# Lukeasargen/Show-Attend-and-Tell-Pytorch-Lightning

Hardware: AMD Instinct MI355X
Metric: captions/sec (train step) at B=128, 256px, seq_len=22 (higher is better)
Workload: dtype bf16; 1 GPU; C2: resnet50 encoder_size=7 encoder_dim=512 vocab=6400 T=22, 128 images/GPU x R=5 captions, trainable encoder, Adam, full lengths, decoder_tf=always; global_batch_images=128, parallelism=dp1, grad_bucket_dtype=fp32

## Files before the change

show-attend-and-tell-pytorch-lightning_amd/csrc/api.hip:

```cpp
#include <stdarg.h>

#include "../../include/sat_hip.h"
#include "decoder.h"
#include "gemm.h"
#include "gemm_bf16_common.h"
#include "temperature.h"
#include "caption_score.h"

namespace sat {
static thread_local char g_err[512] = {0};
int& dev_switch(int which) {
    static int v[SW_COUNT] = {0 , getenv("SAT_NO_WGRAD3X3") ? !atoi(getenv("SAT_NO_WGRAD3X3")) : 1,
                              getenv("SAT_REDUCE_Z16") ? atoi(getenv("SAT_REDUCE_Z16")) : 1, getenv("SAT_WIDE_TILES") ? atoi(getenv("SAT_WIDE_TILES")) : 0,
                              getenv("SAT_BN_ONEPASS") ? atoi(getenv("SAT_BN_ONEPASS")) : 1,
                              getenv("SAT_BN_VPT") ? atoi(getenv("SAT_BN_VPT")) : 2,
                              getenv("SAT_ACC_PREFETCH") ? atoi(getenv("SAT_ACC_PREFETCH")) : 0};
    return v[which];
}
int& trace_launches() { static int on = getenv("SAT_TRACE_LAUNCH") ? 1 : 0; return on; }
char* last_error_buf() { return g_err; }
int fail(int code, const char* fmt, ...) {
    va_list ap; va_start(ap, fmt); vsnprintf(g_err, sizeof g_err, fmt, ap); va_end(ap);
    return code;
}
}

using namespace sat;

extern "C" {

int sat_abi_version(void) { return SAT_HIP_ABI_VERSION; }
int sat_debug_trace_launches(int32_t on) { sat::trace_launches() = on ? 1 : 0; return SAT_OK; }
int sat_debug_option(const char* name, int32_t value) {
    if (!name) return fail(SAT_EINVAL, "debug_option: null name");
    if (!strcmp(name, "wgrad3x3")) { dev_switch(SW_WGRAD3X3) = value; return SAT_OK; }
    if (!strcmp(name, "reduce_z16")) { dev_switch(SW_REDUCE_Z16) = value; return SAT_OK; }
    if (!strcmp(name, "acc_prefetch")) { dev_switch(SW_ACC_PREFETCH) = value; return SAT_OK; }
    if (!strcmp(name, "bn_vpt")) { dev_switch(SW_BN_VPT) = value; return SAT_OK; }
    if (!strcmp(name, "bn_onepass")) { dev_switch(SW_BN_ONEPASS) = value; return SAT_OK; }
    if (!strcmp(name, "wide_tiles")) { dev_switch(SW_WIDE_TILES) = value; return SAT_OK; }
    if (!strcmp(name, "glds_tile")) { glds_force_tile() = value; return SAT_OK; }
    if (!strcmp(name, "glds_stages8")) { glds_stages8() = value; return SAT_OK; }
    if (!strcmp(name, "glds_tall_k")) { glds_tall_k() = value; return SAT_OK; }
    if (!strcmp(name, "glds_tall_conv")) { glds_tall_conv() = value; return SAT_OK; }
    if (!strcmp(name, "tile_override")) { gemm_tile_override() = value; return SAT_OK; }
    return fail(SAT_EINVAL, "debug_option: unknown option %s", name);
}
const char* sat_last_error(void) { return last_error_buf(); }

static int gemm_from_desc(const sat_gemm_desc* d, const sat_gemm_types* t, void* stream);
int sat_gemm_f32(const sat_gemm_desc* d, void* stream) { return gemm_from_desc(d, nullptr, stream); }
int sat_gemm_ex(const sat_gemm_desc* d, const sat_gemm_types* t, void* stream) {
    if (!t) return fail(SAT_EINVAL, "sat_gemm_ex: null type descriptor");
    return gemm_from_desc(d, t, stream);
}
static int gemm_from_desc(const sat_gemm_desc* d, const sat_gemm_types* t, void* stream) {
    if (!d) return fail(SAT_EINVAL, "sat_gemm_f32: null descriptor");
    if (d->amode != A_ROW && d->amode != A_KMAJOR) return fail(SAT_EINVAL, "sat_gemm_f32: amode %d (dense modes only)", d->amode);
    if (d->bmode != B_ROW && d->bmode != B_KMAJOR) return fail(SAT_EINVAL, "sat_gemm_f32: bmode %d (dense modes only)", d->bmode);
    GemmArgs g;
    g.A = d->A; g.lda = d->lda; g.a_rows = d->a_rows; g.B = d->B; g.ldb = d->ldb; g.C = d->C; g.ldc = d->ldc; g.c_rows = d->c_rows;
    g.M = d->M; g.N = d->N; g.K = d->K; g.amode = d->amode; g.bmode = d->bmode; g.accumulate = d->accumulate; g.epi = d->epi;
    g.bias = d->bias; g.e0 = d->e0; g.lde0 = d->lde0; g.c0 = d->c0; g.c1 = d->c1; g.slab = d->slab; g.slab_elems = d->slab_elems;
    if (t) { g.a_bf16 = t->a_bf16; g.b_bf16 = t->b_bf16; g.c_bf16 = t->c_bf16; g.bf16_mfma = t->bf16_mfma; }
    return launch_gemm(g, (hipStream_t)stream);
}

size_t sat_decoder_workspace_bytes(const sat_decoder_dims* d) {
    if (check_dims(d) != SAT_OK) return 0;
    return decoder_workspace_bytes(*d);
}

static int check_params(const sat_decoder_dims* d, const sat_decoder_params* w, const char* what) {
    if (!w) return fail(SAT_EINVAL, "%s: null parameter struct", what);
    if (!w->embedding || !w->init_f_w || !w->init_f_b || !w->init_i_w || !w->init_i_b || !w->w_ih || !w->w_hh || !w->b_ih || !w->b_hh ||
        !w->att_enc || !w->att_dec || !w->att_f || !w->beta_w || !w->beta_b || !w->out_hidden || !w->out_w)
        return fail(SAT_EINVAL, "%s: null tensor in parameter struct", what);
    if (d->deep_output && !w->out_context) return fail(SAT_EINVAL, "%s: deep output needs output.context.weight", what);
    for (int l = 1; l < d->layers; ++l)
        if (!w->up_w_ih[l - 1] || !w->up_w_hh[l - 1] || !w->up_b_ih[l - 1] || !w->up_b_hh[l - 1])
            return fail(SAT_EINVAL, "%s: null tensor for LSTM layer %d", what, l);
    return SAT_OK;
}
static int check_batch(const sat_decoder_batch* b) {
    if (!b || !b->ann || !b->caps || !b->lengths || !b->prow || !b->src_row || !b->step_offsets_host || !b->teacher_host)
        return fail(SAT_EINVAL, "decoder: null field in batch struct");
    return SAT_OK;
}

int sat_decoder_train_fwd(const sat_decoder_dims* d, const sat_decoder_params* w, const sat_decoder_batch* b, float* logits_packed,
                          float* alphas, void* workspace, size_t workspace_bytes, void* stream) {
    SAT_TRY(check_dims(d)); SAT_TRY(check_params(d, w, "decoder_train_fwd")); SAT_TRY(check_batch(b));
    if (!alphas || !workspace || (d->P > 0 && !logits_packed)) return fail(SAT_EINVAL, "decoder_train_fwd: null output/workspace");
    return decoder_fwd(*d, *w, *b, logits_packed, alphas, (char*)workspace, workspace_bytes, (hipStream_t)stream);
}

int sat_decoder_train_bwd(const sat_decoder_dims* d, const sat_decoder_params* w, const sat_decoder_batch* b, const float* dlogits_packed,
                          const float* alphas, const float* dalphas, const sat_decoder_params* g, float* dann, void* workspace,
                          size_t workspace_bytes, void* stream) {
    SAT_TRY(check_dims(d)); SAT_TRY(check_params(d, w, "decoder_train_bwd")); SAT_TRY(check_params(d, g, "decoder_train_bwd(grads)")); SAT_TRY(check_batch(b));
    if (!alphas || !dann || !workspace || (d->P > 0 && !dlogits_packed)) return fail(SAT_EINVAL, "decoder_train_bwd: null input/output/workspace");
    return decoder_bwd(*d, *w, *b, dlogits_packed, alphas, dalphas, *g, dann, (char*)workspace, workspace_bytes, (hipStream_t)stream);
}

int sat_decoder_train_bwd_fork(const sat_decoder_dims* d, const sat_decoder_params* w, const sat_decoder_batch* b, const float* dlogits_packed,
                               const float* alphas, const float* dalphas, const sat_decoder_params* g, float* dann, void* workspace,
                               size_t workspace_bytes, void* side_stream, void* event, void* stream) {
    SAT_TRY(check_dims(d)); SAT_TRY(check_params(d, w, "decoder_train_bwd_fork")); SAT_TRY(check_params(d, g, "decoder_train_bwd_fork(grads)")); SAT_TRY(check_batch(b));
    if (!alphas || !dann || !workspace || (d->P > 0 && !dlogits_packed)) return fail(SAT_EINVAL, "decoder_train_bwd_fork: null input/output/workspace");
    if ((side_stream != nullptr) != (event != nullptr)) return fail(SAT_EINVAL, "decoder_train_bwd_fork: side stream and event go together (got %s only)", side_stream ? "a stream" : "an event");
    if (side_stream && side_stream == stream) return fail(SAT_EINVAL, "decoder_train_bwd_fork: the side stream is the caller's stream");
    if (workspace_bytes < decoder_workspace_bytes(*d))
        return fail(SAT_EINVAL, "decoder_train_bwd_fork: workspace %zu < %zu bytes", workspace_bytes, decoder_workspace_bytes(*d));
    return decoder_bwd(*d, *w, *b, dlogits_packed, alphas, dalphas, *g, dann, (char*)workspace, workspace_bytes, (hipStream_t)stream, (hipStream_t)side_stream,
                       (hipEvent_t)event);
}

int sat_decoder_train_bwd_reg(const sat_decoder_dims* d, const sat_decoder_params* w, const sat_decoder_batch* b, const float* dlogits_packed,
                              const float* alphas, const float* dalphas, const sat_decoder_params* g, float* dann, void* workspace,
                              size_t workspace_bytes, void* side_stream, void* event, void* stream, const float* reg_gscale) {
    if (!reg_gscale)
        return sat_decoder_train_bwd_fork(d, w, b, dlogits_packed, alphas, dalphas, g, dann, workspace, workspace_bytes, side_stream, event, stream);
    SAT_TRY(check_dims(d)); SAT_TRY(check_params(d, w, "decoder_train_bwd_reg")); SAT_TRY(check_params(d, g, "decoder_train_bwd_reg(grads)")); SAT_TRY(check_batch(b));
    if (!alphas || !dann || !workspace || (d->P > 0 && !dlogits_packed)) return fail(SAT_EINVAL, "decoder_train_bwd_reg: null input/output/workspace");
    if ((side_stream != nullptr) != (event != nullptr)) return fail(SAT_EINVAL, "decoder_train_bwd_reg: side stream and event go together (got %s only)", side_stream ? "a stream" : "an event");
    if (side_stream && side_stream == stream) return fail(SAT_EINVAL, "decoder_train_bwd_reg: the side stream is the caller's stream");
    if (workspace_bytes < decoder_workspace_bytes(*d))
        return fail(SAT_EINVAL, "decoder_train_bwd_reg: workspace %zu < %zu bytes", workspace_bytes, decoder_workspace_bytes(*d));
    return decoder_bwd(*d, *w, *b, dlogits_packed, alphas, dalphas, *g, dann, (char*)workspace, workspace_bytes, (hipStream_t)stream, (hipStream_t)side_stream,
                       (hipEvent_t)event, reg_gscale);
}

int sat_decoder_train_reg_fwd(const sat_decoder_dims* d, const sat_decoder_batch* b, void* workspace, size_t workspace_bytes, void* scratch, float* out,
                              void* stream) {
    SAT_TRY(check_dims(d)); SAT_TRY(check_batch(b));
    if (!workspace || !scratch || !out) return fail(SAT_EINVAL, "decoder_train_reg_fwd: null workspace/scratch/out");
    if (workspace_bytes < decoder_workspace_bytes(*d))
        return fail(SAT_EINVAL, "decoder_train_reg_fwd: workspace %zu < %zu bytes", workspace_bytes, decoder_workspace_bytes(*d));
    return decoder_reg_fwd(*d, *b, (char*)workspace, workspace_bytes, scratch, out, (hipStream_t)stream);
}

static int check_activation_reg(const char* what, const void* hidden, const void* lengths, const void* p2, const char* n2, const void* p3, const char* n3,
                                int32_t N, int32_t T1, int32_t n, int64_t P, int64_t Q) {
    if (!hidden || !lengths || !p2 || !p3)
        return fail(SAT_EINVAL, "%s: null pointer (%s)", what, !hidden ? "hidden" : !lengths ? "lengths" : !p2 ? n2 : n3);
    if (N <= 0 || T1 <= 0 || n <= 0) return fail(SAT_EINVAL, "%s: non-positive size (N=%d T1=%d n=%d)", what, N, T1, n);
    if (P < 0 || Q < 0 || Q > P || P > (int64_t)N * T1)
        return fail(SAT_EINVAL, "%s: live counts P=%lld Q=%lld outside 0 <= Q <= P <= N*T1=%lld", what, (long long)P, (long long)Q, (long long)N * T1);
    return SAT_OK;
}
size_t sat_activation_reg_scratch_bytes(int32_t N, int32_t T1, int32_t n) {
    if (N <= 0 || T1 <= 0 || n <= 0) { fail(SAT_EINVAL, "activation_reg_scratch_bytes: non-positive size (N=%d T1=%d n=%d)", N, T1, n); return 0; }
    return activation_reg_scratch_bytes(N, T1, n);
}
int sat_activation_reg_fwd(const float* hidden, const int32_t* lengths, int32_t N, int32_t T1, int32_t n, int64_t P, int64_t Q, void* scratch, float* out,
                           void* stream) {
    SAT_TRY(check_activation_reg("activation_reg_fwd", hidden, lengths, scratch, "scratch", out, "out", N, T1, n, P, Q));
    return activation_reg_fwd(hidden, lengths, N, T1, n, (long)P, (long)Q, scratch, out, (hipStream_t)stream);
}
int sat_activation_reg_bwd(const float* hidden, const int32_t* lengths, int32_t N, int32_t T1, int32_t n, int64_t P, int64_t Q, const float* gscale, float* dH,
                           void* stream) {
    SAT_TRY(check_activation_reg("activation_reg_bwd", hidden, lengths, gscale, "gscale", dH, "dH", N, T1, n, P, Q));
    return activation_reg_bwd(hidden, lengths, N, T1, n, (long)P, (long)Q, gscale, dH, (hipStream_t)stream);
}

int sat_ce_label_smooth_fwd(const float* logits, const int32_t* targets, int32_t P, int32_t V, float smoothing, float* lse_rows,
                            float* loss_rows, int32_t* correct_rows, float* out, void* stream) {
    if (!logits || !targets || !lse_rows || !loss_rows || !correct_rows || !out) return fail(SAT_EINVAL, "ce_label_smooth_fwd: null pointer");
    return ce_fwd(logits, targets, P, V, smoothing, lse_rows, loss_rows, correct_rows, out, (hipStream_t)stream);
}
int sat_ce_label_smooth_bwd(const float* logits, const int32_t* targets, const float* lse_rows, int32_t P, int32_t V, float smoothing,
                            const float* gscale, float* dlogits, void* stream) {
    if (!logits || !targets || !lse_rows || !dlogits) return fail(SAT_EINVAL, "ce_label_smooth_bwd: null pointer");
    return ce_bwd(logits, targets, lse_rows, P, V, smoothing, gscale, dlogits, (hipStream_t)stream);
}
int sat_doubly_stochastic_fwd(const float* alphas, int32_t N, int32_t T1, int32_t L, float gamma, float* asum, float* part, float* out, void* stream) {
    if (!alphas || !asum || !part || !out) return fail(SAT_EINVAL, "doubly_stochastic_fwd: null pointer");
    return ds_fwd(alphas, N, T1, L, gamma, asum, part, out, (hipStream_t)stream);
}
int sat_doubly_stochastic_bwd(const float* asum, const float* gscale, int32_t N, int32_t T1, int32_t L, float gamma, float* dalphas, void* stream) {
    if (!asum || !dalphas) return fail(SAT_EINVAL, "doubly_stochastic_bwd: null pointer");
    return ds_bwd(asum, gscale, N, T1, L, gamma, dalphas, (hipStream_t)stream);
}

size_t sat_temperature_workspace_bytes(int32_t P, int32_t V) {
    if (P <= 0 || V <= 0) { fail(SAT_EINVAL, "temperature_workspace_bytes: non-positive size (P=%d V=%d)", P, V); return 0; }
    return temperature_workspace_bytes(P, V);
// ... 480 lines not shown
```

show-attend-and-tell-pytorch-lightning_amd/csrc/gemm.h:

```cpp
#pragma once
#include "common.h"

namespace sat {

enum AMode : int {
    A_ROW = 0,
    A_KMAJOR = 1,
    A_CONV_FWD = 2,
    A_CONV_DGRAD = 3
};
enum BMode : int {
    B_ROW = 0,
    B_KMAJOR = 1,
    B_CONV_WGRAD = 2,
    B_CONV_DGRAD_W = 3
};
enum Epi : int {
    EPI_NONE = 0,
    EPI_BIAS = 1,
    EPI_BIAS_SIGMOID_RANGE = 2,
    EPI_ADD_TANH = 3,
    EPI_MUL_DTANH = 4,
    EPI_BIAS_RELU = 5
};

struct ConvGeom {
    int N, H, W, C;
    int K, R, S;
    int P, Q;
    int stride, pad;
    int sw = 0;
    int cls = 0, ph = 0, pw = 0, Hc = 0, Wc = 0, r0 = 0, rc = 0, s0 = 0, sc = 0;
};

struct GemmArgs {
    const void* A = nullptr; long lda = 0; const int* a_rows = nullptr;
    const void* B = nullptr; long ldb = 0;
    void* C = nullptr;        long ldc = 0; const int* c_rows = nullptr;
    int a_bf16 = 0, b_bf16 = 0, c_bf16 = 0;
    int bf16_mfma = 0;
    int M = 0, N = 0, K = 0;
    int amode = A_ROW, bmode = B_ROW;
    int accumulate = 0;
    int epi = EPI_NONE;
    const float* bias = nullptr;
    const float* e0 = nullptr; long lde0 = 0;
    int c0 = 0, c1 = 0;
    ConvGeom g = {};
    float* slab = nullptr; long slab_elems = 0;
    const void* bn_x = nullptr; const unsigned char* bn_mask = nullptr; const float* bn_mean = nullptr; const float* bn_invstd = nullptr;
    const void* add_src = nullptr; const unsigned char* add_mask = nullptr;
    float* tile_stats = nullptr; int* tile_rows = nullptr;
};

int launch_gemm(const GemmArgs& a, hipStream_t stream);
int launch_gemm_bf16(const GemmArgs& a, hipStream_t stream);
int gemm_bf16_eligible(const GemmArgs& a);
enum { SW_UNUSED0 = 0, SW_WGRAD3X3 = 1, SW_REDUCE_Z16 = 2, SW_WIDE_TILES = 3, SW_BN_ONEPASS = 4, SW_BN_VPT = 5, SW_ACC_PREFETCH = 6, SW_COUNT = 7 };
int& dev_switch(int which);

int wgrad3x3_eligible(const ConvGeom& g);
int launch_wgrad3x3(const void* dy, const void* x, float* dw, const ConvGeom& g, float* slab, long slab_elems, hipStream_t st);
size_t gemm_slab_bytes(int M, int N, int K);

}
```

show-attend-and-tell-pytorch-lightning_amd/csrc/gemm_bf16_common.h:

```cpp
#pragma once
#include <stdlib.h>

#include "gemm.h"

namespace sat {

typedef __bf16 bf16x8 __attribute__((ext_vector_type(8)));
typedef __bf16 bf16x4 __attribute__((ext_vector_type(4)));
typedef short s16x4 __attribute__((ext_vector_type(4)));
typedef float f32x16 __attribute__((ext_vector_type(16)));

constexpr int NT = 256;

struct BArgs {
    const void* A; long lda; const int* a_rows;
    const void* B; long ldb;
    void* C; long ldc; const int* c_rows;
    int M, N, K;
    int accumulate, epi;
    const float* bias; const float* e0; long lde0; int c0, c1;
    ConvGeom g;
    int kchunk, nsplit;
    float* slab;
    int wide_store;
// ... 321 lines not shown
        __syncthreads();
        constexpr int VPR = BN / 8;
#pragma unroll
        for (int j = 0; j < BM * VPR / NTH; ++j) {
            int v = tid + j * NTH, lr = v / VPR, lc = (v % VPR) * 8;
            int row = bm + lr, col = bn + lc;
            if (row < a.M && col < a.N) {
                bf16x8 o = *reinterpret_cast<const bf16x8*>(cs + lr * LDC + lc);
                const long orow = a.g.cls ? class_row(a, row) : (long)row;
                __bf16* dst = reinterpret_cast<__bf16*>(a.C) + orow * a.ldc + col;
                if (a.accumulate) {
                    const long off = orow * a.ldc + col;
                    bf16x8 old = *reinterpret_cast<const bf16x8*>((a.add_src ? a.add_src : reinterpret_cast<const __bf16*>(a.C)) + off);
                    const unsigned mb = a.add_mask ? (unsigned)a.add_mask[off >> 3] : 0xFFu;
#pragma unroll
                    for (int e = 0; e < 8; ++e) o[e] = (__bf16)((float)o[e] + (((mb >> e) & 1u) ? (float)old[e] : 0.f));
                }
                *reinterpret_cast<bf16x8*>(dst) = o;
                bacc.add(j, o);
            }
        }
        bacc.finish(a, reinterpret_cast<float*>(smem + BM * LDC), bm / BM, bn, tid);
        return;
    }
    if ((a.nsplit > 1) ? a.wide_slab : (sizeof(TC) == 4 && a.wide_store)) {
        constexpr int LDF = BN + 4, RB = BM / WR, VPR = BN / 4;
        float* fs = reinterpret_cast<float*>(smem);
#pragma unroll
        for (int h = 0; h < WR; ++h) {
            __syncthreads();
            if (wrow == h) {
#pragma unroll
                for (int i = 0; i < TM; ++i)
#pragma unroll
                    for (int j = 0; j < TN; ++j)
#pragma unroll
                        for (int r = 0; r < 16; ++r)
                            fs[(i * 32 + (r & 3) + 8 * (r >> 2) + 4 * lh) * LDF + wn + j * 32 + li] = acc[i][j][r];
            }
            __syncthreads();
#pragma unroll
            for (int jj = 0; jj < RB * VPR / NTH; ++jj) {
                const int v = tid + jj * NTH, lr = v / VPR, lc = (v % VPR) * 4;
                const int row = bm + h * RB + lr, col = bn + lc;
                if (row < a.M && col < a.N) {
                    float4 o = *reinterpret_cast<const float4*>(fs + lr * LDF + lc);
                    if (a.nsplit > 1) { *reinterpret_cast<float4*>(a.slab + ((long)bz * a.M + row) * a.N + col) = o; continue; }
                    const long orow = a.g.cls ? class_row(a, row) : (long)row;
                    float* dst = reinterpret_cast<float*>(a.C) + orow * a.ldc + col;
                    if (a.accumulate) { const float4 old = *reinterpret_cast<const float4*>(dst); o.x += old.x; o.y += old.y; o.z += old.z; o.w += old.w; }
                    if (a.epi != EPI_NONE) {
                        o.x = ep_value(a, row, col, o.x); o.y = ep_value(a, row, col + 1, o.y);
                        o.z = ep_value(a, row, col + 2, o.z); o.w = ep_value(a, row, col + 3, o.w);
                    }
                    *reinterpret_cast<float4*>(dst) = o;
                }
            }
        }
        return;
    }
#pragma unroll
    for (int i = 0; i < TM; ++i)
#pragma unroll
        for (int j = 0; j < TN; ++j)
#pragma unroll
            for (int r = 0; r < 16; ++r) {
                int row = bm + wm + i * 32 + (r & 3) + 8 * (r >> 2) + 4 * lh;
                int col = bn + wn + j * 32 + li;
                if (row < a.M && col < a.N) {
                    if (a.nsplit > 1) a.slab[((long)bz * a.M + row) * a.N + col] = acc[i][j][r];
                    else put<TC>(a, row, col, acc[i][j][r]);
                }
            }
}

template <typename TC>
__global__ void splitk_reduce_b_kernel(BArgs a) {
    long idx = (long)blockIdx.x * blockDim.x + threadIdx.x;
    long total = (long)a.M * a.N;
    if (idx >= total) return;
    float v = 0.f;
    for (int z = 0; z < a.nsplit; ++z) v += a.slab[(long)z * total + idx];
    put<TC>(a, (int)(idx / a.N), (int)(idx % a.N), v);
}
template <typename TC>
__global__ void splitk_reduce_b4_kernel(BArgs a) {
    const long idx4 = (long)blockIdx.x * blockDim.x + threadIdx.x;
    const long total4 = (long)a.M * a.N / 4;
    if (idx4 >= total4) return;
    float4 v = make_float4(0.f, 0.f, 0.f, 0.f);
    const float4* s4 = reinterpret_cast<const float4*>(a.slab);
#pragma unroll 4
    for (int z = 0; z < a.nsplit; ++z) { const float4 t = s4[(long)z * total4 + idx4]; v.x += t.x; v.y += t.y; v.z += t.z; v.w += t.w; }
    const long e = idx4 * 4; const int row = (int)(e / a.N), col = (int)(e % a.N);
    if (sizeof(TC) == 4 && a.wide_store && !a.g.cls) {
        float* dst = reinterpret_cast<float*>(a.C) + (long)row * a.ldc + col;
        if (a.accumulate) { const float4 old = *reinterpret_cast<const float4*>(dst); v.x += old.x; v.y += old.y; v.z += old.z; v.w += old.w; }
        if (a.epi != EPI_NONE) { v.x = ep_value(a, row, col, v.x); v.y = ep_value(a, row, col + 1, v.y); v.z = ep_value(a, row, col + 2, v.z); v.w = ep_value(a, row, col + 3, v.w); }
        *reinterpret_cast<float4*>(dst) = v;
    } else {
        put<TC>(a, row, col, v.x); put<TC>(a, row, col + 1, v.y); put<TC>(a, row, col + 2, v.z); put<TC>(a, row, col + 3, v.w);
    }
}

template <typename TC>
__global__ __launch_bounds__(256) void splitk_reduce_z16_kernel(BArgs a) {
    __shared__ float4 part[16][16];
    const int ev = threadIdx.x & 15, zl = threadIdx.x >> 4;
    const long idx4 = (long)blockIdx.x * 16 + ev;
    const long total4 = (long)a.M * a.N / 4;
    float4 v = make_float4(0.f, 0.f, 0.f, 0.f);
    if (idx4 < total4) {
        const float4* s4 = reinterpret_cast<const float4*>(a.slab);
#pragma unroll 4
        for (int z = zl; z < a.nsplit; z += 16) { const float4 t = s4[(long)z * total4 + idx4]; v.x += t.x; v.y += t.y; v.z += t.z; v.w += t.w; }
    }
    part[zl][ev] = v;
    __syncthreads();
    if (zl != 0 || idx4 >= total4) return;
#pragma unroll
    for (int l = 1; l < 16; ++l) { const float4 t = part[l][ev]; v.x += t.x; v.y += t.y; v.z += t.z; v.w += t.w; }
    const long e = idx4 * 4; const int row = (int)(e / a.N), col = (int)(e % a.N);
    if (sizeof(TC) == 4 && a.wide_store && !a.g.cls) {
        float* dst = reinterpret_cast<float*>(a.C) + (long)row * a.ldc + col;
        if (a.accumulate) { const float4 old = *reinterpret_cast<const float4*>(dst); v.x += old.x; v.y += old.y; v.z += old.z; v.w += old.w; }
        if (a.epi != EPI_NONE) { v.x = ep_value(a, row, col, v.x); v.y = ep_value(a, row, col + 1, v.y); v.z = ep_value(a, row, col + 2, v.z); v.w = ep_value(a, row, col + 3, v.w); }
        *reinterpret_cast<float4*>(dst) = v;
    } else {
        put<TC>(a, row, col, v.x); put<TC>(a, row, col + 1, v.y); put<TC>(a, row, col + 2, v.z); put<TC>(a, row, col + 3, v.w);
    }
}

template <typename TC>
inline int launch_splitk_reduce(const BArgs& k, hipStream_t st) {
    const long total = (long)k.M * k.N;
    const int z16 = dev_switch(SW_REDUCE_Z16);
    if (k.wide_slab && z16 && k.nsplit >= 32 && total / 4 / 256 < 256)
        hipLaunchKernelGGL(splitk_reduce_z16_kernel<TC>, dim3(cdiv(total / 4, 16)), dim3(256), 0, st, k);
    else if (k.wide_slab) hipLaunchKernelGGL(splitk_reduce_b4_kernel<TC>, dim3(cdiv(total / 4, 256)), dim3(256), 0, st, k);
    else hipLaunchKernelGGL(splitk_reduce_b_kernel<TC>, dim3(cdiv(total, 256)), dim3(256), 0, st, k);
    return launch_ok("splitk_reduce_b");
}

__device__ __forceinline__ void xcd_tile(int& bx, int& by, int& bz, int y_fastest = 0) {
    const unsigned total = gridDim.x * gridDim.y * gridDim.z;
    const unsigned orig = (blockIdx.z * gridDim.y + blockIdx.y) * gridDim.x + blockIdx.x;
    const unsigned q = total >> 3, r = total & 7, xcd = orig & 7, idx = orig >> 3;
    const unsigned lin = (xcd < r ? xcd * (q + 1) : r * (q + 1) + (xcd - r) * q) + idx;
    if (y_fastest) { by = lin % gridDim.y; const unsigned t2 = lin / gridDim.y; bx = t2 % gridDim.x; bz = t2 / gridDim.x; }
    else { bx = lin % gridDim.x; const unsigned t2 = lin / gridDim.x; by = t2 % gridDim.y; bz = t2 / gridDim.y; }
}

int launch_gemm_glds(const BArgs& k, int amode, int bmode, int c_bf16, int BMt, hipStream_t st, int* bm_used = nullptr);
int& glds_force_tile();
int& glds_stages8();
int& glds_tall_k();
int& glds_tall_conv();
int& glds_ablate();
int& gemm_tile_override();

}
```

show-attend-and-tell-pytorch-lightning_amd/csrc/gemm_glds.hip:

```cpp
#include <stdlib.h>

#include "gemm_bf16_common.h"

namespace sat {

template <int AM, int BMo, typename TC> int glds_run_64(const BArgs& k, hipStream_t st);
template <int AM, int BMo, typename TC> int glds_run_128(const BArgs& k, hipStream_t st);
template <int AM, int BMo, typename TC> int glds_run_128x64(const BArgs& k, hipStream_t st);
#ifdef SAT_DEV_TILES
template <int AM, int BMo, typename TC> int glds_run_256x128(const BArgs& k, hipStream_t st);
template <int AM, int BMo, typename TC> int glds_run_256(const BArgs& k, hipStream_t st);
#endif

enum { TILE_64 = 0, TILE_128 = 1, TILE_128x64 = 2, TILE_256x128 = 3, TILE_256 = 4 };
template <int AM, int BMo, typename TC>
static int rung_tiles(const BArgs& k, int tile, hipStream_t st, int* bm_used) {
    switch (tile) {
#ifdef SAT_DEV_TILES
        case TILE_256: if (bm_used) *bm_used = 256; return glds_run_256<AM, BMo, TC>(k, st);
        case TILE_256x128: if (bm_used) *bm_used = 256; return glds_run_256x128<AM, BMo, TC>(k, st);
#else
        case TILE_256: case TILE_256x128: return -1;
#endif
        case TILE_128: if (bm_used) *bm_used = 128; return glds_run_128<AM, BMo, TC>(k, st);
        case TILE_128x64: if (bm_used) *bm_used = 128; return glds_run_128x64<AM, BMo, TC>(k, st);
        default: if (bm_used) *bm_used = 64; return glds_run_64<AM, BMo, TC>(k, st);
    }
}

int& glds_force_tile() { static int v = getenv("SAT_GLDS_TILE") ? atoi(getenv("SAT_GLDS_TILE")) : -1; return v; }
int& glds_ablate() { static int v = 0; return v; }
int& glds_tall_k() { static int v = getenv("SAT_GLDS_TALL_K") ? atoi(getenv("SAT_GLDS_TALL_K")) : 1 << 30; return v; }
int& glds_tall_conv() { static int v = getenv("SAT_GLDS_TALL_CONV") ? atoi(getenv("SAT_GLDS_TALL_CONV")) : 1152; return v; }
int& glds_stages8() { static int v = getenv("SAT_GLDS_STAGES8") ? atoi(getenv("SAT_GLDS_STAGES8")) : 0; return v; }

int launch_gemm_glds(const BArgs& k0, int amode, int bmode, int c_bf16, int BMt, hipStream_t st, int* bm_used) {
    const int force_tile = glds_force_tile();
    static const int off = getenv("SAT_NO_GLDS") ? atoi(getenv("SAT_NO_GLDS")) : 0;
    static const int force_stages = getenv("SAT_GLDS_STAGES") ? atoi(getenv("SAT_GLDS_STAGES")) : 0;
    static const int deep_from = getenv("SAT_GLDS_DEEP_FROM") ? atoi(getenv("SAT_GLDS_DEEP_FROM")) : 1 << 30;
    static const int rotate = getenv("SAT_GLDS_ROT") ? atoi(getenv("SAT_GLDS_ROT")) : 1 << 20;
    if (off) return -1;
    BArgs k = k0;
    const int ktiles = cdiv(k.kchunk < k.K ? k.kchunk : k.K, 64);
    static const int s1_upto = getenv("SAT_GLDS_S1_UPTO") ? atoi(getenv("SAT_GLDS_S1_UPTO")) : 1 << 30;
    k.nstage = force_stages ? force_stages : (ktiles >= deep_from ? 4 : ((ktiles == 1 || (c_bf16 && ktiles <= s1_upto)) ? 1 : 2));
    k.rotate = rotate;
    if (k.nstage < 1) k.nstage = 1;
    if (k.nstage > 4) k.nstage = 4;
    static const int tall = getenv("SAT_GLDS_TALL") ? atoi(getenv("SAT_GLDS_TALL")) : 2;
    int tile = (BMt >= 256) ? (BMt == 256 ? TILE_256 : TILE_256x128) : (BMt == 128 ? TILE_128 : TILE_64);
    if (tile == TILE_64 && tall && bmode != B_CONV_WGRAD && k.N <= 64 && (amode == A_KMAJOR ? (tall > 1 && k.M >= 128) : k.M >= 8192)) tile = TILE_128x64;
    static const int tall_conv_tiles = getenv("SAT_GLDS_TALL_CONV_TILES") ? atoi(getenv("SAT_GLDS_TALL_CONV_TILES")) : 512;
    if (tile == TILE_128 && bmode != B_CONV_WGRAD && k.nsplit <= 1 &&
        ((amode == A_ROW && k.K <= glds_tall_k()) || ((amode == A_CONV_FWD || amode == A_CONV_DGRAD) && (k.K <= glds_tall_conv() || (long)cdiv(k.M, 128) * cdiv(k.N, 128) < tall_conv_tiles)))) tile = TILE_128x64;
    if (force_tile >= 0) tile = force_tile;
    if (tile == TILE_256 || tile == TILE_256x128) {
        const int maxs = (tile == TILE_256) ? 2 : 3;
        const int deep8 = glds_stages8();
        if (ktiles > 1) k.nstage = deep8 ? (deep8 < maxs ? deep8 : maxs) : (ktiles >= 3 ? maxs : 2);
    }
    {
        static const int order = getenv("SAT_TILE_ORDER") ? atoi(getenv("SAT_TILE_ORDER")) : -1;
        const int tbm = (tile == TILE_64) ? 64 : 128, tbn = (tile == TILE_128) ? 128 : 64;
        const int mt = cdiv(k.M, tbm), nt = cdiv(k.N, tbn);
        k.y_fastest = order >= 0 ? order : (amode == A_ROW && bmode != B_CONV_WGRAD && mt <= 16 && nt >= 2 * mt);
    }
    const ConvGeom& g = k.g;
    if (g.sw && g.sw != g.stride) return -1;
    if (k.K % 64 || k.kchunk % 64 || k.a_rows) return -1;
    if (amode == A_CONV_FWD && (g.C % 64 || g.R * g.S > 32)) return -1;
    if (amode == A_CONV_DGRAD && (g.K % 64 || g.R * g.S > 32 || (g.stride != 1 && !g.cls))) return -1;
    if (bmode == B_CONV_WGRAD && g.R * g.S > 32) return -1;
    const long lim = 1L << 30;
    long a_el = 0, b_el = 0;
    switch (amode) {
        case A_ROW: a_el = (long)k.M * k.lda; break;
        case A_KMAJOR: a_el = (long)k.K * k.lda; break;
        case A_CONV_FWD: a_el = (long)g.N * g.H * g.W * g.C; break;
        default: a_el = (long)g.N * g.P * g.Q * g.K; break;
    }
    switch (bmode) {
        case B_ROW: b_el = (long)k.N * k.ldb; break;
        case B_KMAJOR: b_el = (long)k.K * k.ldb; break;
        case B_CONV_WGRAD: b_el = (long)g.N * g.H * g.W * g.C; break;
        default: b_el = (long)g.K * g.R * g.S * g.C; break;
    }
    if (a_el >= lim || b_el >= lim) return -1;
    if ((amode == A_KMAJOR && k.M < 8) || (bmode != B_ROW && k.N < 8)) return -1;
#define SAT_GCASE(AMV, BMV, TC) return rung_tiles<AMV, BMV, TC>(k, tile, st, bm_used);
    if (amode == A_CONV_FWD && bmode == B_ROW && c_bf16) SAT_GCASE(A_CONV_FWD, B_ROW, __bf16)
    if (amode == A_ROW && bmode == B_ROW && c_bf16) SAT_GCASE(A_ROW, B_ROW, __bf16)
    if (amode == A_ROW && bmode == B_ROW && !c_bf16) SAT_GCASE(A_ROW, B_ROW, float)
    if (amode == A_CONV_DGRAD && bmode == B_CONV_DGRAD_W && c_bf16) SAT_GCASE(A_CONV_DGRAD, B_CONV_DGRAD_W, __bf16)
    if (amode == A_ROW && bmode == B_KMAJOR && c_bf16) SAT_GCASE(A_ROW, B_KMAJOR, __bf16)
    if (amode == A_ROW && bmode == B_KMAJOR && !c_bf16) SAT_GCASE(A_ROW, B_KMAJOR, float)
    if (amode == A_KMAJOR && bmode == B_CONV_WGRAD && !c_bf16) SAT_GCASE(A_KMAJOR, B_CONV_WGRAD, float)
    if (amode == A_KMAJOR && bmode == B_KMAJOR && !c_bf16) SAT_GCASE(A_KMAJOR, B_KMAJOR, float)
#undef SAT_GCASE
    return -1;
}

}
```

Before: 32680 captions/s.

## Add intra-block wave split-K GEMM kernel for small fp32 output GEMMs

Result: no change. 32990 captions/s (median of 6 runs) (+1.0%).

```diff
diff --git a/show-attend-and-tell-pytorch-lightning_amd/csrc/api.hip b/show-attend-and-tell-pytorch-lightning_amd/csrc/api.hip
--- a/show-attend-and-tell-pytorch-lightning_amd/csrc/api.hip
+++ b/show-attend-and-tell-pytorch-lightning_amd/csrc/api.hip
@@ -10,7 +10,7 @@
 namespace sat {
 static thread_local char g_err[512] = {0};
 int& dev_switch(int which) {
-    static int v[SW_COUNT] = {0 , getenv("SAT_NO_WGRAD3X3") ? !atoi(getenv("SAT_NO_WGRAD3X3")) : 1,
+    static int v[SW_COUNT] = {getenv("SAT_GLDS_WAVE_SPLIT") ? atoi(getenv("SAT_GLDS_WAVE_SPLIT")) : 1, getenv("SAT_NO_WGRAD3X3") ? !atoi(getenv("SAT_NO_WGRAD3X3")) : 1,
                               getenv("SAT_REDUCE_Z16") ? atoi(getenv("SAT_REDUCE_Z16")) : 1, getenv("SAT_WIDE_TILES") ? atoi(getenv("SAT_WIDE_TILES")) : 0,
                               getenv("SAT_BN_ONEPASS") ? atoi(getenv("SAT_BN_ONEPASS")) : 1,
                               getenv("SAT_BN_VPT") ? atoi(getenv("SAT_BN_VPT")) : 2,
@@ -33,6 +33,7 @@
 int sat_debug_trace_launches(int32_t on) { sat::trace_launches() = on ? 1 : 0; return SAT_OK; }
 int sat_debug_option(const char* name, int32_t value) {
     if (!name) return fail(SAT_EINVAL, "debug_option: null name");
+    if (!strcmp(name, "wave_split")) { dev_switch(SW_WAVE_SPLIT) = value; return SAT_OK; }
     if (!strcmp(name, "wgrad3x3")) { dev_switch(SW_WGRAD3X3) = value; return SAT_OK; }
     if (!strcmp(name, "reduce_z16")) { dev_switch(SW_REDUCE_Z16) = value; return SAT_OK; }
     if (!strcmp(name, "acc_prefetch")) { dev_switch(SW_ACC_PREFETCH) = value; return SAT_OK; }
diff --git a/show-attend-and-tell-pytorch-lightning_amd/csrc/gemm.h b/show-attend-and-tell-pytorch-lightning_amd/csrc/gemm.h
--- a/show-attend-and-tell-pytorch-lightning_amd/csrc/gemm.h
+++ b/show-attend-and-tell-pytorch-lightning_amd/csrc/gemm.h
@@ -56,7 +56,7 @@
 int launch_gemm(const GemmArgs& a, hipStream_t stream);
 int launch_gemm_bf16(const GemmArgs& a, hipStream_t stream);
 int gemm_bf16_eligible(const GemmArgs& a);
-enum { SW_UNUSED0 = 0, SW_WGRAD3X3 = 1, SW_REDUCE_Z16 = 2, SW_WIDE_TILES = 3, SW_BN_ONEPASS = 4, SW_BN_VPT = 5, SW_ACC_PREFETCH = 6, SW_COUNT = 7 };
+enum { SW_WAVE_SPLIT = 0, SW_WGRAD3X3 = 1, SW_REDUCE_Z16 = 2, SW_WIDE_TILES = 3, SW_BN_ONEPASS = 4, SW_BN_VPT = 5, SW_ACC_PREFETCH = 6, SW_COUNT = 7 };
 int& dev_switch(int which);
 
 int wgrad3x3_eligible(const ConvGeom& g);
diff --git a/show-attend-and-tell-pytorch-lightning_amd/csrc/gemm_bf16_common.h b/show-attend-and-tell-pytorch-lightning_amd/csrc/gemm_bf16_common.h
--- a/show-attend-and-tell-pytorch-lightning_amd/csrc/gemm_bf16_common.h
+++ b/show-attend-and-tell-pytorch-lightning_amd/csrc/gemm_bf16_common.h
@@ -497,6 +497,8 @@
 }
 
 int launch_gemm_glds(const BArgs& k, int amode, int bmode, int c_bf16, int BMt, hipStream_t st, int* bm_used = nullptr);
+constexpr int WAVE_SPLIT_ROWS = 32;
+int glds_run_wave_split(const BArgs& k, hipStream_t st);
 int& glds_force_tile();
 int& glds_stages8();
 int& glds_tall_k();
diff --git a/show-attend-and-tell-pytorch-lightning_amd/csrc/gemm_glds.hip b/show-attend-and-tell-pytorch-lightning_amd/csrc/gemm_glds.hip
--- a/show-attend-and-tell-pytorch-lightning_amd/csrc/gemm_glds.hip
+++ b/show-attend-and-tell-pytorch-lightning_amd/csrc/gemm_glds.hip
@@ -33,6 +33,14 @@
 int& glds_tall_k() { static int v = getenv("SAT_GLDS_TALL_K") ? atoi(getenv("SAT_GLDS_TALL_K")) : 1 << 30; return v; }
 int& glds_tall_conv() { static int v = getenv("SAT_GLDS_TALL_CONV") ? atoi(getenv("SAT_GLDS_TALL_CONV")) : 1152; return v; }
 int& glds_stages8() { static int v = getenv("SAT_GLDS_STAGES8") ? atoi(getenv("SAT_GLDS_STAGES8")) : 0; return v; }
+static int cu_count() {
+    static const int n = [] {
+        int dev = 0, v = 0;
+        if (hipGetDevice(&dev) != hipSuccess || hipDeviceGetAttribute(&v, hipDeviceAttributeMultiprocessorCount, dev) != hipSuccess) v = 0;
+        return v;
+    }();
+    return n;
+}
 
 int launch_gemm_glds(const BArgs& k0, int amode, int bmode, int c_bf16, int BMt, hipStream_t st, int* bm_used) {
     const int force_tile = glds_force_tile();
@@ -88,6 +96,11 @@
     }
     if (a_el >= lim || b_el >= lim) return -1;
     if ((amode == A_KMAJOR && k.M < 8) || (bmode != B_ROW && k.N < 8)) return -1;
+    if (dev_switch(SW_WAVE_SPLIT) && tile == TILE_64 && amode == A_ROW && bmode == B_KMAJOR && !c_bf16 && !k.c_rows && !g.cls && !k.tile_stats &&
+        k.nsplit >= 2 && k.nsplit <= 4 && k.wide_slab && k.wide_store && (long)cdiv(k.M, WAVE_SPLIT_ROWS) * cdiv(k.N, 64) <= cu_count()) {
+        if (bm_used) *bm_used = 64;
+        return glds_run_wave_split(k, st);
+    }
 #define SAT_GCASE(AMV, BMV, TC) return rung_tiles<AMV, BMV, TC>(k, tile, st, bm_used);
     if (amode == A_CONV_FWD && bmode == B_ROW && c_bf16) SAT_GCASE(A_CONV_FWD, B_ROW, __bf16)
     if (amode == A_ROW && bmode == B_ROW && c_bf16) SAT_GCASE(A_ROW, B_ROW, __bf16)
diff --git a/show-attend-and-tell-pytorch-lightning_amd/csrc/gemm_glds_t64ws.hip b/show-attend-and-tell-pytorch-lightning_amd/csrc/gemm_glds_t64ws.hip
--- /dev/null
+++ b/show-attend-and-tell-pytorch-lightning_amd/csrc/gemm_glds_t64ws.hip
@@ -0,0 +1,222 @@
+#include "gemm_glds_kernel.h"
+
+namespace sat {
+
+__device__ __forceinline__ unsigned lds_addr(const void* p) { return (unsigned)(size_t)(lptr_t)p; }
+__device__ __forceinline__ bf16x8 lds_read_b128(const __bf16* p) {
+    bf16x8 v = {};
+#if defined(__HIP_DEVICE_COMPILE__)
+    asm volatile("ds_read_b128 %0, %1" : "=v"(v) : "v"(lds_addr(p)));
+#endif
+    return v;
+}
+__device__ __forceinline__ bf16x4 lds_read_tr16_b64(const __bf16* p) {
+    bf16x4 v = {};
+#if defined(__HIP_DEVICE_COMPILE__)
+    asm volatile("ds_read_b64_tr_b16 %0, %1" : "=v"(v) : "v"(lds_addr(p)));
+#endif
+    return v;
+}
+__device__ __forceinline__ void lds_reads_done() { asm volatile("s_waitcnt lgkmcnt(0)" ::: "memory"); }
+template <typename T> __device__ __forceinline__ void lds_use(T& v) {
+#if defined(__HIP_DEVICE_COMPILE__)
+    asm volatile("" : "+v"(v));
+#endif
+}
+
+template <int BM, int S>
+__global__ __launch_bounds__(256, 1) void gemm_glds_ws_kernel(BArgs a) {
+    constexpr int KB = 64, BN = 64;
+    constexpr int A_EL = BM * KB, B_EL = BN * KB, STAGE = A_EL + B_EL;
+    constexpr int NA = BM / 8, NB = BN / 8, G = NA + NB;
+    constexpr int TM = BM / 32, TN = 2;
+    constexpr int LDF = BN + 4;
+    static_assert(BM * LDF * 4 <= S * STAGE * 2, "the fp32 tile is staged in the wave's own ring");
+    static_assert(S == 2 || S == 3, "ring depth");
+    extern __shared__ __attribute__((aligned(1024))) __bf16 smem[];
+
+    const int tid = threadIdx.x, lane = tid & 63;
+    const int z = __builtin_amdgcn_readfirstlane(tid >> 6);
+    int bx, by, bz;
+    xcd_tile(bx, by, bz, a.y_fastest);
+    const int bm = by * BM, bn = bx * BN;
+    const int kbeg = z * a.kchunk;
+    const int kend = min(a.K, kbeg + a.kchunk);
+    const int li = lane & 31, lh = lane >> 5;
+    const int tg = lane >> 4, ti = lane & 15;
+    const int t_h = tg >> 1, t_mh = tg & 1, t_q = ti >> 2, t_p = ti & 3;
+    const i32x4 rA = make_rsrc(a.A), rB = make_rsrc(a.B);
+    __bf16* ring = smem + z * S * STAGE;
+    const int by64 = (by * BM) >> 6;
+
+    int a_off0[NA], b_off0[NB];
+#pragma unroll
+    for (int j = 0; j < NA; ++j) {
+        const int row = j * 8 + (lane >> 3), ks = (lane & 7) ^ ((row >> 1) & 7);
+        int m = bm + row;
+        if (m >= a.M) m = a.M - 1;
+        a_off0[j] = (int)(((long)m * a.lda + ks * 8) * 2);
+    }
+#pragma unroll
+    for (int j = 0; j < NB; ++j) {
+        const int krow = j * 8 + (lane >> 3), sl = lane & 7;
+        const int lq = (sl >> 2) ^ ((krow >> 1) & 1);
+        int n = bn + (lq * 4 + (sl & 3)) * 8;
+        if (n >= a.N) n = a.N - 8;
+        b_off0[j] = (int)(((long)krow * a.ldb + n) * 2);
+    }
+
+    const int T = (kend - kbeg + KB - 1) / KB;
+    int tcur = (T > 0 && a.rotate) ? (int)((unsigned)(bx * 5 + by64 * 3 + z) % (unsigned)(T < a.rotate ? T : a.rotate)) : 0;
+    int sA = 0, sB = 0;
+    auto seek = [&](int tile) {
+        const int k0 = kbeg + tile * KB;
+        sA = k0 * 2;
+        sB = (int)((long)k0 * a.ldb * 2);
+    };
+    seek(tcur);
+    auto advance_tile = [&]() {
+        if (++tcur == T) { tcur = 0; seek(0); return; }
+        sA += KB * 2;
+        sB += (int)(KB * a.ldb * 2);
+    };
+    auto issue_piece = [&](int buf, int jj) {
+        __bf16* as = ring + buf * STAGE; __bf16* bs = as + A_EL;
+#pragma unroll
+        for (int j = 0; j < NA; ++j) if (j == jj) dma16(rA, a_off0[j], sA, as + j * 512);
+#pragma unroll
+        for (int j = 0; j < NB; ++j) if (j + NA == jj) dma16(rB, b_off0[j], sB, bs + j * 512);
+    };
+
+    f32x16 acc[TM][TN];
+#pragma unroll
+    for (int i = 0; i < TM; ++i)
+#pragma unroll
+        for (int j = 0; j < TN; ++j)
+#pragma unroll
+            for (int r = 0; r < 16; ++r) acc[i][j][r] = 0.f;
+
+    int a_off[TM], a_sw[TM], b_off[TN];
+#pragma unroll
+    for (int i = 0; i < TM; ++i) { const int row = i * 32 + li; a_off[i] = row * KB; a_sw[i] = (row >> 1) & 7; }
+#pragma unroll
+    for (int j = 0; j < TN; ++j) {
+        const int col = j * 32 + 16 * t_mh + 4 * t_p, kr = 8 * t_h + t_q;
+        const int sw = (kr >> 1) & 1;
+        b_off[j] = kr * BN + (((col >> 5) ^ sw) << 5) + (col & 31);
+    }
+
+    if (T > 0) {
+        for (int t = 0; t < S - 1 && t < T; ++t) {
+#pragma unroll
+            for (int jj = 0; jj < G; ++jj) issue_piece(t, jj);
+            advance_tile();
+        }
+        int cur = 0, nxt = S - 1;
+        for (int it = 0; it < T; ++it) {
+            if (S == 3 && it + 1 < T) asm volatile("s_waitcnt vmcnt(%0)" ::"n"(G) : "memory");
+            else asm volatile("s_waitcnt vmcnt(0)" ::: "memory");
+            __builtin_amdgcn_sched_barrier(0);
+            const bool more = it + S - 1 < T;
+            const __bf16* as = ring + cur * STAGE;
+            const __bf16* bs = as + A_EL;
+            bf16x8 af[KB / 16][TM], bf[KB / 16][TN];
+            bf16x4 blo[KB / 16][TN], bhi[KB / 16][TN];
+#pragma unroll
+            for (int ks = 0; ks < KB / 16; ++ks) {
+                const int kk = ks * 16;
+#pragma unroll
+                for (int i = 0; i < TM; ++i) af[ks][i] = lds_read_b128(as + a_off[i] + ((((kk >> 3) + lh) ^ a_sw[i]) << 3));
+#pragma unroll
+                for (int j = 0; j < TN; ++j) {
+                    const __bf16* p = bs + b_off[j] + kk * BN;
+                    blo[ks][j] = lds_read_tr16_b64(p); bhi[ks][j] = lds_read_tr16_b64(p + 4 * BN);
+                }
+            }
+            if (more) {
+#pragma unroll
+                for (int jj = 0; jj < G / 4; ++jj) issue_piece(nxt, jj);
+            }
+            lds_reads_done();
+#pragma unroll
+            for (int ks = 0; ks < KB / 16; ++ks) {
+#pragma unroll
+                for (int i = 0; i < TM; ++i) lds_use(af[ks][i]);
+#pragma unroll
+                for (int j = 0; j < TN; ++j) {
+                    lds_use(blo[ks][j]); lds_use(bhi[ks][j]);
+                    bf[ks][j] = __builtin_shufflevector(blo[ks][j], bhi[ks][j], 0, 1, 2, 3, 4, 5, 6, 7);
+                }
+            }
+#pragma unroll
+            for (int ks = 0; ks < KB / 16; ++ks) {
+                if (more && ks > 0) {
+#pragma unroll
+                    for (int jj = (ks * G) / 4; jj < ((ks + 1) * G) / 4; ++jj) issue_piece(nxt, jj);
+                }
+#pragma unroll
+                for (int i = 0; i < TM; ++i)
+#pragma unroll
+                    for (int j = 0; j < TN; ++j)
+                        acc[i][j] = __builtin_amdgcn_mfma_f32_32x32x16_bf16(af[ks][i], bf[ks][j], acc[i][j], 0, 0, 0);
+            }
+            if (more) advance_tile();
+            cur = (cur + 1 == S) ? 0 : cur + 1;
+            nxt = (nxt + 1 == S) ? 0 : nxt + 1;
+        }
+    }
+
+    float* fs = reinterpret_cast<float*>(ring);
+    if (z < a.nsplit) {
+#pragma unroll
+        for (int i = 0; i < TM; ++i)
+#pragma unroll
+            for (int j = 0; j < TN; ++j)
+#pragma unroll
+                for (int r = 0; r < 16; ++r) fs[(i * 32 + (r & 3) + 8 * (r >> 2) + 4 * lh) * LDF + j * 32 + li] = acc[i][j][r];
+    }
+    __syncthreads();
+    constexpr int VPR = BN / 4, WSTRIDE = S * STAGE / 2;
+    const float* f0 = reinterpret_cast<const float*>(smem);
+#pragma unroll
+    for (int jj = 0; jj < BM * VPR / 256; ++jj) {
+        const int v = tid + jj * 256, lr = v / VPR, lc = (v % VPR) * 4;
+        const int row = bm + lr, col = bn + lc;
+        if (row < a.M && col < a.N) {
+            float4 o = make_float4(0.f, 0.f, 0.f, 0.f);
+            for (int s = 0; s < a.nsplit; ++s) {
+                const float4 t = *reinterpret_cast<const float4*>(f0 + s * WSTRIDE + lr * LDF + lc);
+                o.x += t.x; o.y += t.y; o.z += t.z; o.w += t.w;
+            }
+            float* dst = reinterpret_cast<float*>(a.C) + (long)row * a.ldc + col;
+            if (a.accumulate) { const float4 old = *reinterpret_cast<const float4*>(dst); o.x += old.x; o.y += old.y; o.z += old.z; o.w += old.w; }
+            if (a.epi != EPI_NONE) {
+                o.x = ep_value(a, row, col, o.x); o.y = ep_value(a, row, col + 1, o.y);
+                o.z = ep_value(a, row, col + 2, o.z); o.w = ep_value(a, row, col + 3, o.w);
+            }
+            *reinterpret_cast<float4*>(dst) = o;
+        }
+    }
+}
+
+int glds_run_wave_split(const BArgs& k, hipStream_t st) {
+    constexpr int BM = WAVE_SPLIT_ROWS, S = 3;
+    dim3 grid(cdiv(k.N, 64), cdiv(k.M, BM), 1);
+    char pname[128];
+    if (profile_enabled()) {
+        static const bool shapes = getenv("SAT_PROFILE_SHAPES") != nullptr;
+        if (shapes) snprintf(pname, sizeof pname, "gemm_glds_nn_64x64 M%d N%d K%d z%d", k.M, k.N, k.K, k.nsplit);
+        else snprintf(pname, sizeof pname, "gemm_glds_nn_64x64");
+    }
+    ProfScope prof(pname, 2.0 * k.M * k.N * k.K, 2.0 * k.M * k.K + 2.0 * k.N * k.K + 4.0 * k.M * k.N, st);
+    constexpr size_t lds = (size_t)4 * S * (BM + 64) * 64 * sizeof(__bf16);
+    static bool attr_set = false;
+    if (!attr_set) {
+        SAT_CHECK_HIP(hipFuncSetAttribute(reinterpret_cast<const void*>(&gemm_glds_ws_kernel<BM, S>), hipFuncAttributeMaxDynamicSharedMemorySize, (int)lds));
+        attr_set = true;
+    }
+    hipLaunchKernelGGL((gemm_glds_ws_kernel<BM, S>), grid, dim3(256), lds, st, k);
+    return launch_ok("gemm_glds_ws_kernel");
+}
+
+}
```
